# ewrfcas/LeftRefill

Hardware: AMD Instinct MI355X
Metric: 512x1024 stitched images/sec @ 50 DDIM steps, cfg=2.5; per-UNet-step ms (higher is better)
Workload: dtype f16; 1 GPU; configs[1]: 1-ref inpainting, 512x1024 canvas (latent 64x128), B=4 per GPU (UNet batch 8 under CFG), 50 DDIM steps, cfg=2.5, eta=1.0, fp16; global_batch=4, per_gpu_batch=4, ddim_steps=50, parallelism=dp1 (sample-sharded, no data-path collective), ranks=1

## Files before the change

include/leftrefill_hip.h:

```cpp
#ifndef LEFTREFILL_HIP_H
#define LEFTREFILL_HIP_H

#include <stdint.h>

#ifdef __cplusplus
extern "C" {
#endif

#define LR_E_ARG (-1)
#define LR_E_ALIGN (-2)
#define LR_E_UNSUPPORTED (-3)

typedef void* lr_stream_t;
typedef uint16_t lr_half;
#define LR_DTYPE_F16 0
#define LR_DTYPE_BF16 1
#define LR_PIPE_DEFAULT 0
#define LR_PIPE_W8_DEEP 4
#define LR_PIPE_HALO 8

int lr_abi_version(void);

int lr_nchw_f32_to_nhwc_f16(const float* x1, int C1, const float* x2, int C2, lr_half* y, int Cpad, int N, int H,
                            int W, lr_stream_t s);
// ... 45 lines not shown
  int32_t dtype;
  int32_t pipe;
  float* gn_group_out; int32_t gn_hw;
  int32_t wt_bstride, bias_bstride;
  int32_t wt_pm;
  const lr_half* skip1; const lr_half* skip2; int32_t Cs1, Cs2;
  int32_t splitk_mode;
} lr_gemm_args;
int lr_gemm_gn_group_chunks(const lr_gemm_args* args);
int lr_gemm_gn_rows(const lr_gemm_args* args);
int lr_gemm_plan(const lr_gemm_args* args, int32_t* plan);
int lr_gemm_stats_parts(const lr_gemm_args* args);
int64_t lr_gemm_workspace_bytes(const lr_gemm_args* args);
int lr_gemm_conv_f16(const lr_gemm_args* args, lr_stream_t s);
int lr_gemm_splitk_timeouts(void);

int lr_attention_f16(const lr_half* q, int ldq, const lr_half* k, int ldk, const lr_half* v, int ldv, lr_half* o,
                     int ldo, int B, int heads, int Nq, int Nkv, float scale, lr_stream_t s);

int lr_attention_causal_f16(const lr_half* q, int ldq, const lr_half* k, int ldk, const lr_half* v, int ldv, lr_half* o,
                            int ldo, int B, int heads, int N, float scale, lr_stream_t s);
int lr_attention_vt_f16(const lr_half* q, int ldq, const lr_half* k, int ldk, const lr_half* vt, int ld_vt, lr_half* o,
                        int ldo, int B, int heads, int Nq, int Nkv, float scale, lr_stream_t s);
int lr_transpose_v_f16(const lr_half* v, int ldv, lr_half* vt, int ld_vt, int B, int heads, int Nkv, lr_stream_t s);

typedef struct lr_xattn_args {
  const lr_half* x; lr_half* out;
  const lr_half* wq; const float* bq;
  const lr_half* k; int32_t ldk;
  const lr_half* vt;
// ... 215 lines not shown
```

leftrefill_amd/_lib.py:

```python
import ctypes
import os

HERE = os.path.dirname(os.path.abspath(__file__))
LIB_PATH = os.environ.get("LEFTREFILL_LIB_PATH") or os.path.join(HERE, "lib", "libleftrefill_hip.so")
ABI_VERSION = 30

c_void_p, c_int, c_float, c_int64 = ctypes.c_void_p, ctypes.c_int, ctypes.c_float, ctypes.c_int64


class GemmArgs(ctypes.Structure):
    _fields_ = [
        ("p1", c_void_p), ("C1", ctypes.c_int32),
        ("p2", c_void_p), ("C2", ctypes.c_int32),
        ("B", ctypes.c_int32), ("H", ctypes.c_int32), ("W", ctypes.c_int32),
        ("Hs", ctypes.c_int32), ("Ws", ctypes.c_int32),
        ("taps", ctypes.c_int32), ("stride", ctypes.c_int32), ("up", ctypes.c_int32),
        ("asym", ctypes.c_int32),
        ("wt", c_void_p), ("N", ctypes.c_int32),
        ("bias", c_void_p),
        ("rowvec", c_void_p), ("ld_rowvec", ctypes.c_int32),
        ("resid", c_void_p), ("ld_resid", ctypes.c_int32),
        ("out", c_void_p), ("ld_out", ctypes.c_int32),
        ("geglu", ctypes.c_int32),
        ("tile_n", ctypes.c_int32),
        ("tile_m", ctypes.c_int32),
        ("splits", ctypes.c_int32),
        ("workspace", c_void_p), ("workspace_bytes", ctypes.c_int64),
        ("ln_stats", c_void_p), ("ln_parts", ctypes.c_int32), ("ln_eps", ctypes.c_float),
        ("ln_colsum", c_void_p),
        ("stats_out", c_void_p),
        ("gn_stats_out", c_void_p),
        ("dtype", ctypes.c_int32),
        ("pipe", ctypes.c_int32),
        ("gn_group_out", c_void_p), ("gn_hw", ctypes.c_int32),
        ("wt_bstride", ctypes.c_int32), ("bias_bstride", ctypes.c_int32),
        ("wt_pm", ctypes.c_int32),
        ("skip1", c_void_p), ("skip2", c_void_p), ("Cs1", ctypes.c_int32), ("Cs2", ctypes.c_int32),
        ("splitk_mode", ctypes.c_int32),
    ]


class AttnBwdArgs(ctypes.Structure):
    _fields_ = ([(n, c_void_p) for n in ("q", "k", "v", "o", "dout", "qt", "kt", "dot", "lse", "dsum", "dq", "dk", "dv")] +
                [(n, ctypes.c_int32) for n in ("ldq", "ldk", "ldv", "ldo", "lddo", "ld_qt", "ld_kt", "lddq", "lddk", "lddv",
                                               "B", "heads", "Nq", "Nkv")] + [("scale", ctypes.c_float)])


class XattnArgs(ctypes.Structure):
    _fields_ = [("x", c_void_p), ("out", c_void_p), ("wq", c_void_p), ("bq", c_void_p), ("k", c_void_p), ("ldk", ctypes.c_int32),
                ("vt", c_void_p), ("wo", c_void_p), ("bo", c_void_p), ("stats_out", c_void_p),
                ("M", ctypes.c_int32), ("HW", ctypes.c_int32), ("C", ctypes.c_int32), ("heads", ctypes.c_int32),
                ("Lc", ctypes.c_int32), ("ln_eps", ctypes.c_float), ("scale", ctypes.c_float),
                ("pre_a", c_void_p), ("pre_w", c_void_p), ("pre_b", c_void_p)]

# ... 86 lines not shown
    "lr_ddim_cfg_step": [c_void_p, c_void_p, c_int, c_void_p, c_void_p, c_void_p, c_int64, c_float, c_float, c_float,
                         c_float, c_float, c_void_p],
    "lr_timestep_embedding_f32": [c_void_p, c_int, c_int, c_void_p, c_void_p],
    "lr_plms_cfg_step": [c_void_p, c_void_p, c_int, c_void_p, c_int, c_void_p, c_float, c_void_p, c_void_p, c_void_p, c_int64,
                         c_float, c_float, c_float, c_float, c_void_p],
    "lr_dpmpp_cfg_step": [c_void_p, c_void_p, c_int, c_void_p, c_void_p, c_void_p, c_int64, c_float, c_float, c_float, c_float,
                          c_float, c_float, c_float, c_void_p],
    "lr_ddim_inv_cfg_step": [c_void_p, c_void_p, c_int, c_void_p, c_int64, c_float, c_float, c_float, c_void_p],
    "lr_ddim_cfg3_step": [c_void_p, c_void_p, c_int, c_void_p, c_void_p, c_void_p, c_int64, c_float, c_float, c_float, c_float,
                          c_float, c_float, c_float, c_void_p],
    "lr_ddpm_step": [c_void_p, c_void_p, c_int, c_void_p, c_void_p, c_void_p, c_void_p, c_int64, c_int64, c_int, c_void_p, c_void_p,
                     c_int64, c_float, c_float, c_float, c_float, c_float, c_float, c_float, c_void_p],
    "lr_ddim_q_sample": [c_void_p, c_void_p, c_void_p, c_int, c_int64, c_void_p, c_void_p, c_void_p],
    "lr_eval_metrics": [c_void_p, c_int, c_void_p, c_void_p, c_int, c_int, c_int, c_int, c_int, c_int, c_void_p, c_void_p, c_void_p,
                        c_void_p],
}

BF16_TWINS = ["lr_groupnorm_stats", "lr_groupnorm_apply", "lr_groupnorm_apply_n", "lr_layernorm", "lr_layernorm_bwd",
              "lr_groupnorm_bwd", "lr_layernorm_bwd_res", "lr_groupnorm_bwd_res", "lr_nchw_f32_to_nhwc_f16", "lr_nhwc_f16_to_nchw", "lr_timestep_embedding", "lr_linear_small_m",
              "lr_mv_gather", "lr_mv_scatter", "lr_ddim_cfg_step", "lr_timestep_embedding_f32", "lr_plms_cfg_step",
              "lr_dpmpp_cfg_step", "lr_ddim_inv_cfg_step", "lr_ddim_cfg3_step", "lr_ddpm_step", "lr_geglu_fwd", "lr_geglu_bwd", "lr_sumpool2x2",
              "lr_mv_gather_bwd", "lr_mv_scatter_bwd", "lr_attention_f16", "lr_attention_causal_f16", "lr_attention_lse_f16",
              "lr_attention_vt_f16", "lr_transpose_v_f16", "lr_attention_bwd_f16", "lr_xattn_block_f16",
              "lr_xattn_pack_vt_f16", "lr_ffn_block_f16", "lr_stin_block_f16", "lr_rowlin_f16", "lr_gn_conv_out_f16",
              "lr_attention_causal_lse_f16", "lr_attention_causal_bwd_f16", "lr_gelu_fwd_f16", "lr_gelu_bwd_f16"]


def twin(name):
    return (name[:-4] if name.endswith("_f16") else name) + "_bf16"

# ... 67 lines not shown
```

leftrefill_amd/csrc/gemm_conv.hip:

```cpp
#include "gemm_common.h"
#include <atomic>

#ifdef LR_GEMM_TRACE
static unsigned long long* g_trace = nullptr;
extern "C" void lr_gemm_set_trace(void* p) { g_trace = (unsigned long long*)p; }
#endif


template <int BN, int MODE, typename T>
__global__ __launch_bounds__(GEMM_THREADS, BN == 64 ? 4 : BN == 128 ? 3 : 2) void gemm_conv_kernel(const GemmParams P) {
#if defined(__HIP_DEVICE_COMPILE__)
  constexpr int TM = 4;
  constexpr int TN = BN / 32;
  constexpr int A_BYTES = BM * 128;
  constexpr int B_BYTES = BN * 128;
  constexpr int STAGE = A_BYTES + B_BYTES;
  extern __shared__ __attribute__((aligned(16))) char smem[];

  const int t = threadIdx.x;
  const int lane = t & 63;
  const int w = __builtin_amdgcn_readfirstlane(t >> 6);
  const int wm = w >> 1, wn = w & 1;
#ifdef LR_GEMM_STAGGER
  if (P.stagger) {
// ... 622 lines not shown
      if (t < 2 * (8 * RED_GROUPS / gcg)) {
        const int gl = t >> 1, j = t & 1;
        const int g = (blockIdx.x * 8 * RED_GROUPS) / gcg + gl;
        if (g < 32) {
          float a = 0.f;
          for (int c = 0; c < gcg; ++c) a += red[j][gl * gcg + c];
          const int m0 = blockIdx.y * RED_ROWS;
          const int smp = m0 / P.gp_hw, chunk = (m0 - smp * P.gp_hw) / RED_ROWS;
          P.gp_out[(((size_t)smp * P.gp_chunks + chunk) * 32 + g) * 2 + j] = a;
        }
      }
    }
  }
}

template <int BN, int MODE, typename T>
static int launch_gemm_t(const GemmParams& P0, hipStream_t st) {
  GemmParams P = P0;
  P.ntiles_n = (P.N + BN - 1) / BN;
  const int ntm = (P.M + BM - 1) / BM;
  P.ntiles_m = ntm;
  P.m_fastest = 0;
  P.nblocks = P.ntiles_n * ntm;
  const size_t smem = 2 * (size_t)(BM + BN) * 128 + BM * 2 * sizeof(float) + 2 * (((BN + 63) / 64) * 64) * sizeof(float);
  static unsigned long long attr_done = 0;
  if (lr_attr_needed(&attr_done)) {
    hipFuncSetAttribute(reinterpret_cast<const void*>(gemm_conv_kernel<BN, MODE, T>), hipFuncAttributeMaxDynamicSharedMemorySize,
                        (int)smem);
  }
  hipLaunchKernelGGL((gemm_conv_kernel<BN, MODE, T>), dim3(P.nblocks, P.splits), dim3(GEMM_THREADS), smem, st, P);
// ... 147 lines not shown
  if (!base[dev]) {
    void* p = nullptr;
    if (hipGetSymbolAddress(&p, HIP_SYMBOL(lr_sk_counters)) != hipSuccess) return nullptr;
    base[dev] = (unsigned*)p;
  }
  return base[dev] + (size_t)(next.fetch_add(1, std::memory_order_relaxed) & 15) * 2048;
}

extern "C" int lr_gemm_splitk_timeouts(void) {
  unsigned v = 0;
  if (hipMemcpyFromSymbol(&v, HIP_SYMBOL(lr_sk_error), sizeof(v)) != hipSuccess) return -1;
  const unsigned h = lr_halo_sk_timeouts();
  return h == 0xFFFFFFFFu ? -1 : (int)(v + h);
}

extern "C" int lr_gemm_conv_f16(const lr_gemm_args* a, lr_stream_t s) {
  if (!a || !a->p1 || !a->wt || !a->out) return LR_E_ARG;
  GemmParams P;
  P.p1 = (const f16*)a->p1; P.C1 = a->C1;
  P.p2 = (const f16*)a->p2; P.C2 = a->p2 ? a->C2 : 0;
  P.c16 = (P.C1 == 16 && P.C2 == 0 && a->taps == 9 && a->stride == 1 && a->up == 0 && !a->asym) ? 1 : 0;
  if (P.C1 <= 0 || (!P.c16 && P.C1 % 64) || P.C2 % 64) return LR_E_ALIGN;
  if (a->taps != 1 && a->taps != 9) return LR_E_UNSUPPORTED;
  if (a->stride != 1 && a->stride != 2) return LR_E_UNSUPPORTED;
  if (a->up < 0 || a->up > 2) return LR_E_UNSUPPORTED;
  if (a->B <= 0 || a->H <= 0 || a->W <= 0 || a->Hs <= 0 || a->Ws <= 0 || a->N <= 0) return LR_E_ARG;
  P.H = a->H; P.W = a->W; P.Hs = a->Hs; P.Ws = a->Ws;
  P.taps = a->taps; P.stride = a->stride; P.up = a->up;
  P.zins = (a->up == 2) ? 1 : 0;
  if (P.zins) P.up = 1;
  P.pad = a->asym ? 0 : 1;
  P.wt = (const f16*)a->wt; P.N = a->N; P.bias = a->bias;
// ... 79 lines not shown
    if (P.gp_chunks <= 0 || ((uintptr_t)P.gp_out & 7) || a->stats_out) return LR_E_ARG;
    P.gp_cg = P.N / 32;
    P.gp_hw = a->gn_hw > 0 ? a->gn_hw : a->H * a->W;
  }
  P.wt_pm = a->wt_pm ? 1 : 0;
  if (P.wt_pm && (a->wt_bstride || P.K % 64)) return LR_E_ARG;
  P.wt_bstride = a->wt_bstride; P.bias_bstride = a->bias_bstride;
  if (P.wt_bstride) {
    if (a->taps != 1 || splits > 1 || P.rows_per_batch % tm || P.wt_bstride < 0 || P.bias_bstride < 0 || (P.wt_bstride & 7)) return LR_E_ARG;
    if ((int64_t)a->B * P.wt_bstride * 2 >= lim) return LR_E_UNSUPPORTED;
  }
  P.st_out = a->stats_out;
  P.st_parts = ((P.N + tn - 1) / tn) * tile_wnw(tm, tn, P.geglu);
  if (P.st_out && (splits > 1 || ((uintptr_t)P.st_out & 7))) return LR_E_ARG;
  hipStream_t st = (hipStream_t)s;
  int rc;
  const int mode = P.geglu ? 1 : P.gelu ? 2 : 0;
  if (a->pipe != 0 && a->pipe != choose_stages(tm, tn, a->pipe)) return LR_E_UNSUPPORTED;
  const bool deep = tm == 128 && choose_stages(tm, tn, a->pipe) == 4;
#ifdef LR_DEV_VARIANTS
  if (P.splits > 1 && a->splitk_mode == 1 && mode != 1 && (tn == 160 || tn == 320) && (tm == 256 || deep || a->pipe == LR_PIPE_HALO)) {
    const int64_t tiles = (int64_t)((P.M + tm - 1) / tm) * ((P.N + tn - 1) / tn);
    if (tiles * P.splits <= 256 && tiles <= 2048 && (int64_t)P.splits * P.M * P.N * 4 < lim && P.N % 8 == 0)
      P.sk_cnt = sk_counter_slot();
  }
#endif
  if (a->pipe == LR_PIPE_HALO) {
    if (mode != 0 || a->asym) return LR_E_UNSUPPORTED;
    rc = lr_launch_conv_halo(P, tn, st);
    if (rc || P.splits == 1 || P.sk_cnt) return rc;
    return launch_reduce(P, st);
  }
  if (mode == 0) {
    if (deep && tn == 128) rc = launch_pipe<128, 8, 128, 4, 4, 0>(P, st);
    else if (deep && tn == 160) rc = launch_pipe<128, 8, 160, 4, 4, 0>(P, st);

    else if (tm == 128 && tn == 128) rc = launch_gemm<128, 0>(P, st);
    else if (tm == 128 && tn == 64) rc = launch_gemm<64, 0>(P, st);
    else if (tm == 128 && tn == 160) rc = launch_gemm<160, 0>(P, st);
    else if (tm == 256 && tn == 128) rc = launch_gemm256<128, 4, 3, 0>(P, st);
    else if (tm == 256 && tn == 160) rc = launch_gemm256<160, 4, 3, 0>(P, st);
    else if (tm == 256 && tn == 256) rc = launch_gemm256<256, 2, 2, 0>(P, st);
    else if (tm == 256 && tn == 320) rc = launch_gemm256<320, 2, 2, 0>(P, st);
    else return LR_E_UNSUPPORTED;
  } else if (mode == 1) {
    if (deep && tn == 128) rc = launch_pipe<128, 8, 128, 4, 4, 1>(P, st);
    else if (deep) return LR_E_UNSUPPORTED;
    else if (tm == 128 && tn == 128) rc = launch_gemm<128, 1>(P, st);
    else if (tm == 128 && tn == 64) rc = launch_gemm<64, 1>(P, st);
    else if (tm == 256 && tn == 128) rc = launch_gemm256<128, 4, 3, 1>(P, st);
    else if (tm == 256 && tn == 256) rc = launch_gemm256<256, 2, 2, 1>(P, st);
    else if (tm == 256 && tn == 320) rc = launch_gemm256<320, 4, 2, 1>(P, st);
    else return LR_E_UNSUPPORTED;
  } else {
    if (deep) return LR_E_UNSUPPORTED;
    if (tm == 128 && tn == 128) rc = launch_gemm<128, 2>(P, st);
    else if (tm == 128 && tn == 64) rc = launch_gemm<64, 2>(P, st);
    else if (tm == 256 && tn == 128) rc = launch_gemm256<128, 4, 3, 2>(P, st);
    else return LR_E_UNSUPPORTED;
  }
  if (rc || P.splits == 1 || P.sk_cnt) return rc;
  return launch_reduce(P, st);
}
```

leftrefill_amd/csrc/stin_block.hip:

```cpp
#include "chain_common.h"

#define SI_C 320
#define SI_ROWS 256
#define SI_THREADS 512
#define SI_SLOT 40960
#define SI_OUT_AUX 0

struct StinParams {
  const void* x; const void* wp; const float* bp; const void* wqkv; const float* bqkv;
  void* x1; void* qkv;
  int M, NQ, ld_qkv;
  float eps;
  const float* gn_part; const float* gn_gamma; const float* gn_beta; int gn_chunks, gn_hw; float gn_eps;
#ifdef SI_TRACE
  unsigned long long* trace;
#endif
};

#ifdef SI_TRACE
#define SI_STAMP(k) do { if (P.trace && lane == 0) P.trace[((size_t)blockIdx.x * 8 + w) * 64 + (k)] = __builtin_readcyclecounter(); } while (0)
static unsigned long long* g_si_trace = nullptr;
extern "C" void lr_stin_set_trace(void* p) { g_si_trace = (unsigned long long*)p; }
#else
#define SI_STAMP(k) do { } while (0)
// ... 231 lines not shown
  if ((int64_t)a->NQ * SI_C * 2 >= ((int64_t)1 << 31)) return LR_E_UNSUPPORTED;
  StinParams P;
  P.x = a->x; P.wp = a->wp; P.bp = a->bp; P.wqkv = a->wqkv; P.bqkv = a->bqkv; P.x1 = a->x1; P.qkv = a->qkv;
  P.M = a->M; P.NQ = a->NQ; P.ld_qkv = a->ld_qkv; P.eps = a->ln_eps;
  const bool gn = a->gn_part != nullptr;
  if (gn) {
    if (!a->gn_gamma || !a->gn_beta || a->gn_chunks <= 0 || a->gn_hw <= 0) return LR_E_ARG;
    if (a->gn_hw % SI_ROWS || a->M % a->gn_hw) return LR_E_UNSUPPORTED;
    if (((uintptr_t)a->gn_part & 7) || (((uintptr_t)a->gn_gamma | (uintptr_t)a->gn_beta) & 3)) return LR_E_ALIGN;
  }
  P.gn_part = a->gn_part; P.gn_gamma = a->gn_gamma; P.gn_beta = a->gn_beta; P.gn_chunks = a->gn_chunks; P.gn_hw = a->gn_hw; P.gn_eps = a->gn_eps;
#ifdef SI_TRACE
  P.trace = g_si_trace;
#endif
  const size_t smem = 3 * SI_SLOT + (size_t)(SI_C + a->NQ + 2 * SI_C + 64) * sizeof(float);
  static unsigned long long attr_done[2] = {0, 0};
  if (gn) {
    if (lr_attr_needed(&attr_done[1]))
      hipFuncSetAttribute(reinterpret_cast<const void*>(stin_block_kernel<T, true>), hipFuncAttributeMaxDynamicSharedMemorySize, (int)smem);
    hipLaunchKernelGGL((stin_block_kernel<T, true>), dim3(a->M / SI_ROWS), dim3(SI_THREADS), smem, (hipStream_t)s, P);
  } else {
    if (lr_attr_needed(&attr_done[0]))
      hipFuncSetAttribute(reinterpret_cast<const void*>(stin_block_kernel<T, false>), hipFuncAttributeMaxDynamicSharedMemorySize, (int)smem);
    hipLaunchKernelGGL((stin_block_kernel<T, false>), dim3(a->M / SI_ROWS), dim3(SI_THREADS), smem, (hipStream_t)s, P);
  }
  return lr_launch_status();
}

extern "C" int lr_stin_block_f16(const lr_stin_args* a, lr_stream_t s) { return stin_block_t<f16>(a, s); }
extern "C" int lr_stin_block_bf16(const lr_stin_args* a, lr_stream_t s) { return stin_block_t<bf16>(a, s); }
```

leftrefill_amd/engine.py:

```python
import math
from dataclasses import dataclass
from typing import Optional

import torch

from . import packing
from . import train_ops as ops
from .ops import plan_batch_scale

_COMPUTE = [torch.float16]


def compute_dtype():
    return _COMPUTE[0]


class compute:

    def __init__(self, dtype):
        if dtype not in (torch.float16, torch.bfloat16):
            raise ValueError(f"compute dtype must be float16 or bfloat16, got {dtype}")
        self.dtype = dtype

    def __enter__(self):
# ... 1 lines not shown
        _COMPUTE[0] = self.dtype

    def __exit__(self, *exc):
        _COMPUTE[0] = self.prev


@dataclass
class Act:
    tok: torch.Tensor
    N: int
    H: int
    W: int
    tok2: Optional[torch.Tensor] = None
    gs: Optional[tuple] = None
    gs2: Optional[tuple] = None

    @property
    def HW(self):
        return self.H * self.W

    def materialize(self):
        if self.tok2 is None:
            return self.tok
        return torch.cat([self.tok, self.tok2], dim=1).contiguous()


def f32(p):
    return p.detach().float().contiguous()


# ... 163 lines not shown


def ln_linear(x, st, pn: PackedNorm, pl: PackedLinear, wide=None):
    if wide and pl.wf is not None and fold_ok(x) and ops.rowlin_ok(x.shape[0], x.shape[1], pl.wf.shape[0], wide):
        return ops.rowlin(x, pl.wf, pl.bf, eps=pl.eps)
    if st is not None and pl.wf is not None and fold_ok(x):
        return ops.gemm_conv(x, pl.wf, B=1, H=1, W=x.shape[0], taps=1, bias=pl.bf, ln=(st, pl.eps, pl.cs))
    return linear(ops.layer_norm(x, pn.g, pn.b, pn.eps), pl)


GN_FUSE = __import__("os").environ.get("LEFTREFILL_GN_FUSE", "1") != "0"
SKIP_FUSED = __import__("os").environ.get("LEFTREFILL_SKIP_FUSED", "1") != "0"
FF_PROJ = __import__("os").environ.get("LEFTREFILL_FF_PROJ", "1") != "0"


def gn_fuse_ok(x):
    return GN_FUSE and not (torch.is_grad_enabled() and x.requires_grad)


TRAIN_GN_STATS = __import__("os").environ.get("LEFTREFILL_TRAIN_GN_STATS", "1") != "0"
TRAIN_FORK = __import__("os").environ.get("LEFTREFILL_TRAIN_FORK", "1") != "0"


TRAIN_SKIP_FUSED = __import__("os").environ.get("LEFTREFILL_TRAIN_SKIP_FUSED", "1") != "0"


def gn_stats_ok(x):
    return GN_FUSE and (TRAIN_GN_STATS or not torch.is_grad_enabled())


def training(x):
    return torch.is_grad_enabled() and x.requires_grad


def forking(x):
    return TRAIN_FORK and training(x)


def conv(act: Act, pc: PackedConv, rowvec=None, resid=None, up=0, asym=False, gn_stats=False, skip=None, skip_parts=None):
    if pc.taps == 9:
        if up:
            H, W = act.H * 2, act.W * 2
        elif pc.stride == 2:
            H, W = act.H // 2, act.W // 2
        else:
            H, W = act.H, act.W
    else:
        H, W = act.H, act.W
    want = gn_stats and gn_stats_ok(act.tok) and pc.cout == pc.w.shape[0]
    extra = {} if skip_parts is None else {"skip_parts": skip_parts}
    y = ops.gemm_conv(act.tok, pc.w, B=act.N, H=H, W=W, Hs=act.H, Ws=act.W, taps=pc.taps, stride=pc.stride, up=up,
                      asym=asym, x2=act.tok2, bias=pc.b, rowvec=rowvec, resid=resid, want_gn_stats=want, skip=skip, **extra)
    y, gs = y if want else (y, None)
    return Act(y, act.N, H, W, gs=gs)


def _gn_train_stats(act: Act):
    HW = act.HW
    if not (act.gs is not None and HW % act.gs[1] == 0 and gn_stats_ok(act.tok)
            and (act.tok2 is None or (act.gs2 is not None and HW % act.gs2[1] == 0))):
        return None
    if act.tok2 is None and act.gs[2] is not None:
        return ("groups", act.gs[2], act.gs[3])
    return ("channels", act.gs, act.gs2)


def gn(act: Act, pn: PackedNorm, silu):
    HW = act.HW
    if training(act.tok) or (act.tok2 is not None and training(act.tok2)):
        return Act(ops.group_norm(act.tok, act.N, HW, pn.g, pn.b, pn.eps, silu, act.tok2, stats=_gn_train_stats(act)), act.N, act.H, act.W)
    fused = (act.gs is not None and HW % act.gs[1] == 0 and gn_fuse_ok(act.tok)
             and (act.tok2 is None or (act.gs2 is not None and HW % act.gs2[1] == 0)))
    if fused and act.tok2 is None and act.gs[2] is not None:
        y = ops.group_norm_groups(act.tok, act.N, HW, pn.g, pn.b, pn.eps, silu, act.gs[2], act.gs[3])
    elif fused:
        y = ops.group_norm_fused(act.tok, act.N, HW, pn.g, pn.b, pn.eps, silu, act.gs, act.tok2, act.gs2)
    else:
        y = ops.group_norm(act.tok, act.N, HW, pn.g, pn.b, pn.eps, silu, act.tok2)
    return Act(y, act.N, act.H, act.W)


def gn_fork(act: Act, pn: PackedNorm, silu):
    y, t1, t2 = ops.group_norm_fork(act.tok, act.N, act.HW, pn.g, pn.b, pn.eps, silu, act.tok2, stats=_gn_train_stats(act))
    return Act(y, act.N, act.H, act.W), Act(t1, act.N, act.H, act.W, tok2=t2)


def resblock(act: Act, pr: PackedRes, emb_out):
    if forking(act.tok) or (act.tok2 is not None and forking(act.tok2)):
        h, act = gn_fork(act, pr.n1, True)
    else:
        h = gn(act, pr.n1, True)
    h = conv(h, pr.c1, rowvec=emb_out, gn_stats=True)
    h = gn(h, pr.n2, True)
    if pr.c2s is not None and SKIP_FUSED and gn_fuse_ok(act.tok) and gn_fuse_ok(h.tok) and (act.tok2 is None or gn_fuse_ok(act.tok2)):
        return conv(h, pr.c2s, gn_stats=True, skip=(act.tok, act.tok2))
    if (pr.c2s is not None and SKIP_FUSED and TRAIN_SKIP_FUSED and (training(h.tok) or training(act.tok) or (act.tok2 is not None and training(act.tok2)))
            and h.tok2 is None):
        return conv(h, pr.c2s, gn_stats=True, skip=(act.tok, act.tok2), skip_parts=(pr.c2.w, pr.skip.w))
    if pr.skip is not None:
        resid = conv(act, pr.skip).tok
    else:
        resid = act.materialize()
    return conv(h, pr.c2, resid=resid, gn_stats=True)


def attention_plain(x, ctx, pa: PackedAttn, B, L, Lc=None):
    if pa.is_self:
# ... 336 lines not shown
```

leftrefill_amd/ops.py:

```python
import ctypes
import os

import torch

from . import _lib
from ._lib import FfnArgs, GemmArgs, RowlinArgs, StinArgs, XattnArgs

GN_CHUNKS = 256
GN_GROUPS = os.environ.get("LEFTREFILL_GN_GROUPS", "1") != "0"

AUTOTUNE = os.environ.get("LEFTREFILL_AUTOTUNE", "0") == "1"
TILE_CANDIDATES = ((128, 64, 0), (128, 128, 0), (128, 160, 0), (128, 128, 4), (128, 160, 4), (256, 128, 0), (256, 160, 0),
                   (256, 256, 0), (256, 320, 0), (256, 160, 8), (256, 320, 8))
TILE_TABLE_PATH = os.environ.get("LEFTREFILL_TILE_TABLE_PATH",
                                 os.path.join(os.path.dirname(os.path.abspath(__file__)), "tile_table.json"))
_tile_cache = None
PLAN_LOG = os.environ.get("LEFTREFILL_PLAN_LOG", "0") == "1"
SPLITK_MODE = int(os.environ.get("LEFTREFILL_SPLITK_MODE", "0"))
_untabulated = set()
TABLE_HITS, TABLE_MISSES = set(), set()
PLAN_TRIAL = None
LAUNCH_HOOK = None


# ... 179 lines not shown
    _chk16(a, "a")
    _chk16(w, "w")
    M, K = a.shape
    N = w.shape[0]
    out = torch.empty(M, N, device=a.device, dtype=a.dtype)
    st = _stream()
    for m0 in range(0, M, 16):
        mc = min(16, M - m0)
        _lib.check(_fn(lib, "lr_linear_small_m", a.dtype)(a[m0:].data_ptr(), K, _p(w), _p(bias), out[m0:].data_ptr(), N, mc, N, K,
                                         int(act_in), int(act_out), st), "linear_small_m")
    return out


def gemm_conv(x1, wt, *, B, H, W, Hs=None, Ws=None, taps=1, stride=1, up=0, asym=False, x2=None, bias=None, rowvec=None,
              resid=None, geglu=False, gelu=False, out=None, tile_n=0, tile_m=0, splits=0, pipe=0, ln=None,
              want_stats=False, want_gn_stats=False, gn_hw=0, per_sample=False, wt_pm=False, skip=None):
    lib = _lib.load()
    _chk16(x1, "x1")
    _chk16(wt, "wt")
    Hs = H if Hs is None else Hs
    Ws = W if Ws is None else Ws
    C1 = x1.shape[-1]
    C2 = 0
    if x2 is not None:
        _chk16(x2, "x2")
        C2 = x2.shape[-1]
    if per_sample:
        assert wt.dim() == 3 and wt.shape[0] == B and taps == 1 and x2 is None and wt.is_contiguous() and not wt_pm
    if wt_pm:
        assert wt.dim() == 3 and wt.shape[2] == 64 and wt.is_contiguous()
        Nw, Kw = wt.shape[1], wt.shape[0] * 64
# ... 78 lines not shown
                a.pipe = 0
        if skip is not None and best is None:
            plan = (ctypes.c_int32 * 4)()
            lib.lr_gemm_plan(a, plan)
            a.tile_m, a.tile_n, a.splits, a.pipe = plan[0], plan[1], plan[2], plan[3]
    stats = None
    if want_stats:
        if a.splits == 0:
            a.splits = 1
        parts = lib.lr_gemm_stats_parts(a)
        stats = torch.empty(M, parts, 2, device=x1.device, dtype=torch.float32)
        a.stats_out = _p(stats)
    if ln is not None and a.splits == 0:
        a.splits = 1
    gstats = None
    if want_gn_stats:
        plan = (ctypes.c_int32 * 4)()
        lib.lr_gemm_plan(a, plan)
        a.splits = plan[2]
        rows = lib.lr_gemm_gn_rows(a)
        hw = gn_hw or H * W
        if hw % rows == 0:
            chunks = lib.lr_gemm_gn_group_chunks(a) if GN_GROUPS else 0
            gp = torch.empty(M // hw, chunks, 32, 2, device=x1.device, dtype=torch.float32) if chunks > 0 else None
            gstats = (torch.empty((M + rows - 1) // rows, n_out, 2, device=x1.device, dtype=torch.float32), rows, gp, chunks)
            a.gn_stats_out = _p(gstats[0])
            a.gn_group_out = _p(gp)
    ws = _workspace(lib, a, x1.device)
    if LAUNCH_HOOK is not None and tile_m == 0 and tile_n == 0 and splits == 0:
        plan = (ctypes.c_int32 * 4)()
        lib.lr_gemm_plan(a, plan)
        LAUNCH_HOOK(key, 0, tuple(plan))
        rc = lib.lr_gemm_conv_f16(a, st)
        LAUNCH_HOOK(key, 1, rc)
        if rc != 0 and PLAN_TRIAL is not None and PLAN_TRIAL.get(key) is not None:
            PLAN_TRIAL[key] = None
            return gemm_conv(x1, wt, B=B, H=H, W=W, Hs=Hs, Ws=Ws, taps=taps, stride=stride, up=up, asym=asym, x2=x2, bias=bias, rowvec=rowvec,
                             resid=resid, geglu=geglu, gelu=gelu, out=out, ln=ln, want_stats=want_stats, want_gn_stats=want_gn_stats, gn_hw=gn_hw,
                             per_sample=per_sample, wt_pm=wt_pm, skip=skip)
        _lib.check(rc, "gemm_conv")
    else:
        _lib.check(lib.lr_gemm_conv_f16(a, st), "gemm_conv")
    if want_gn_stats:
        return out, gstats
    return (out, stats) if want_stats else out


HEURISTIC_REFINE = os.environ.get("LEFTREFILL_HEURISTIC_REFINE", "1") != "0"


def _lib_plan(lib, a):
    plan = (ctypes.c_int32 * 4)()
    lib.lr_gemm_plan(a, plan)
    return tuple(plan)


def _refine_plan(lib, a, act_epilogue):
    base = _lib_plan(lib, a)
    tm, tn = base[0], base[1]
    M = a.B * a.H * a.W
# ... 472 lines not shown
```

Baseline: 4.781 images/s.

## Fuse split-K reduction with following GroupNorm+SiLU in ResBlock conv1

Adds a split-K reduce kernel that sums the partials, applies bias, rowvec and residual, keeps the per-sample tile in shared memory, computes GroupNorm statistics and writes the normalized SiLU output directly. ResBlock conv1 uses it when eligible (hw<=512, split-K planned) and skips writing the raw conv output, removing the separate GN apply pass and one activation round trip. The cost is one block per sample per 40 channels, which may limit parallelism, plus double-precision stat reduction. It also raises the stin_block dynamic shared-memory attribute to a fixed maximum.

```diff
diff --git a/include/leftrefill_hip.h b/include/leftrefill_hip.h
--- a/include/leftrefill_hip.h
+++ b/include/leftrefill_hip.h
@@ -83,6 +83,27 @@
 int64_t lr_gemm_workspace_bytes(const lr_gemm_args* args);
 int lr_gemm_conv_f16(const lr_gemm_args* args, lr_stream_t s);
 int lr_gemm_splitk_timeouts(void);
+
+typedef struct lr_reduce_gn_args {
+  const float* partials; int32_t splits, M, N;
+  int32_t hw;
+  const float* bias;
+  const lr_half* rowvec; int32_t ld_rowvec;
+  const lr_half* resid; int32_t ld_resid;
+  lr_half* raw; int32_t ld_raw;
+  const float* gamma; const float* beta; float eps; int32_t silu;
+  lr_half* y;
+  float* gn_group_out;
+  int32_t dtype;
+} lr_reduce_gn_args;
+int lr_splitk_reduce_gn(const lr_reduce_gn_args* args, lr_stream_t s);
+int lr_splitk_reduce(const lr_reduce_gn_args* args, lr_stream_t s);
+typedef struct lr_gn_consumer {
+  const float* gamma; const float* beta; float eps; int32_t silu;
+  lr_half* y;
+} lr_gn_consumer;
+int lr_gemm_conv_gn_f16(const lr_gemm_args* args, const lr_gn_consumer* gn, lr_stream_t s);
+int lr_gemm_reduce_gn_ok(const lr_gemm_args* args);
 
 int lr_attention_f16(const lr_half* q, int ldq, const lr_half* k, int ldk, const lr_half* v, int ldv, lr_half* o,
                      int ldo, int B, int heads, int Nq, int Nkv, float scale, lr_stream_t s);
diff --git a/leftrefill_amd/_lib.py b/leftrefill_amd/_lib.py
--- a/leftrefill_amd/_lib.py
+++ b/leftrefill_amd/_lib.py
@@ -38,6 +38,17 @@
         ("skip1", c_void_p), ("skip2", c_void_p), ("Cs1", ctypes.c_int32), ("Cs2", ctypes.c_int32),
         ("splitk_mode", ctypes.c_int32),
     ]
+
+
+class ReduceGnArgs(ctypes.Structure):
+    _fields_ = [("partials", c_void_p), ("splits", ctypes.c_int32), ("M", ctypes.c_int32), ("N", ctypes.c_int32), ("hw", ctypes.c_int32),
+                ("bias", c_void_p), ("rowvec", c_void_p), ("ld_rowvec", ctypes.c_int32), ("resid", c_void_p), ("ld_resid", ctypes.c_int32),
+                ("raw", c_void_p), ("ld_raw", ctypes.c_int32), ("gamma", c_void_p), ("beta", c_void_p), ("eps", ctypes.c_float),
+                ("silu", ctypes.c_int32), ("y", c_void_p), ("gn_group_out", c_void_p), ("dtype", ctypes.c_int32)]
+
+
+class GnConsumer(ctypes.Structure):
+    _fields_ = [("gamma", c_void_p), ("beta", c_void_p), ("eps", ctypes.c_float), ("silu", ctypes.c_int32), ("y", c_void_p)]
 
 
 class AttnBwdArgs(ctypes.Structure):
@@ -154,6 +165,10 @@
     "lr_ddim_q_sample": [c_void_p, c_void_p, c_void_p, c_int, c_int64, c_void_p, c_void_p, c_void_p],
     "lr_eval_metrics": [c_void_p, c_int, c_void_p, c_void_p, c_int, c_int, c_int, c_int, c_int, c_int, c_void_p, c_void_p, c_void_p,
                         c_void_p],
+    "lr_splitk_reduce_gn": [ctypes.POINTER(ReduceGnArgs), c_void_p],
+    "lr_splitk_reduce": [ctypes.POINTER(ReduceGnArgs), c_void_p],
+    "lr_gemm_conv_gn_f16": [ctypes.POINTER(GemmArgs), ctypes.POINTER(GnConsumer), c_void_p],
+    "lr_gemm_reduce_gn_ok": [ctypes.POINTER(GemmArgs)],
 }
 
 BF16_TWINS = ["lr_groupnorm_stats", "lr_groupnorm_apply", "lr_groupnorm_apply_n", "lr_layernorm", "lr_layernorm_bwd",
diff --git a/leftrefill_amd/csrc/gemm_conv.hip b/leftrefill_amd/csrc/gemm_conv.hip
--- a/leftrefill_amd/csrc/gemm_conv.hip
+++ b/leftrefill_amd/csrc/gemm_conv.hip
@@ -660,6 +660,162 @@
   }
 }
 
+#define RG_OCT 5
+#define RG_CH (8 * RG_OCT)
+#define RG_ROWS 128
+#define RG_THREADS (RG_OCT * RG_ROWS)
+#define RG_MAX_HW 512
+#define RG_MAX_CHUNKS (RG_MAX_HW / RED_ROWS)
+struct ReduceGnParams {
+  const float* ws; int splits, M, N, hw;
+  const float* bias; const void* rowvec; int ld_rowvec; const void* resid; int ld_resid;
+  void* raw; int ld_raw;
+  const float* gamma; const float* beta; float eps; int silu; void* y;
+};
+
+template <typename T>
+__global__ __launch_bounds__(RG_THREADS) void splitk_reduce_gn_kernel(const ReduceGnParams P) {
+  __shared__ uint4 rows[RG_MAX_HW * RG_OCT];
+  __shared__ float chs[RG_MAX_CHUNKS][RG_CH][2];
+  __shared__ float gps[RG_MAX_CHUNKS][4][2];
+  __shared__ float s_mean[4], s_rstd[4];
+  const int t = threadIdx.x, o = t % RG_OCT, r = t / RG_OCT;
+  const int ncb = P.N / RG_CH, total = gridDim.x;
+  const int vb = total % 8 == 0 ? (blockIdx.x % 8) * (total / 8) + blockIdx.x / 8 : blockIdx.x;
+  const int smp = vb / ncb, n = (vb - smp * ncb) * RG_CH + o * 8;
+  const int Cg = P.N / 32, ngl = RG_CH / Cg, nchunks = P.hw / RED_ROWS;
+  const size_t slice = (size_t)P.M * P.N;
+  const T* rowvec = (const T*)P.rowvec;
+  const T* resid = (const T*)P.resid;
+  float add[8];
+  float rv[8];
+#pragma unroll
+  for (int i = 0; i < 8; ++i) { add[i] = P.bias ? P.bias[n + i] : 0.f; rv[i] = 0.f; }
+  if (rowvec) lr_unpack8<T>(*reinterpret_cast<const uint4*>(rowvec + (size_t)smp * P.ld_rowvec + n), rv);
+  for (int row = r; row < P.hw; row += RG_ROWS) {
+    const size_t m = (size_t)smp * P.hw + row;
+    const float* src = P.ws + m * P.N + n;
+    float v[8];
+#pragma unroll
+    for (int i = 0; i < 8; ++i) v[i] = 0.f;
+    int sidx = 0;
+    for (; sidx + 4 <= P.splits; sidx += 4) {
+      f32x4 a[4], b[4];
+#pragma unroll
+      for (int k = 0; k < 4; ++k) {
+        a[k] = *reinterpret_cast<const f32x4*>(src + (sidx + k) * slice);
+        b[k] = *reinterpret_cast<const f32x4*>(src + (sidx + k) * slice + 4);
+      }
+#pragma unroll
+      for (int k = 0; k < 4; ++k) {
+        v[0] += a[k][0]; v[1] += a[k][1]; v[2] += a[k][2]; v[3] += a[k][3];
+        v[4] += b[k][0]; v[5] += b[k][1]; v[6] += b[k][2]; v[7] += b[k][3];
+      }
+    }
+    for (; sidx < P.splits; ++sidx) {
+      const f32x4 a = *reinterpret_cast<const f32x4*>(src + sidx * slice), b = *reinterpret_cast<const f32x4*>(src + sidx * slice + 4);
+      v[0] += a[0]; v[1] += a[1]; v[2] += a[2]; v[3] += a[3]; v[4] += b[0]; v[5] += b[1]; v[6] += b[2]; v[7] += b[3];
+    }
+    if (P.bias) {
+#pragma unroll
+      for (int i = 0; i < 8; ++i) v[i] += add[i];
+    }
+    if (rowvec) {
+#pragma unroll
+      for (int i = 0; i < 8; ++i) v[i] += rv[i];
+    }
+    if (resid) {
+      float e[8];
+      lr_unpack8<T>(*reinterpret_cast<const uint4*>(resid + m * P.ld_resid + n), e);
+#pragma unroll
+      for (int i = 0; i < 8; ++i) v[i] += e[i];
+    }
+    const uint4 pk = lr_pack8<T>(v);
+    rows[row * RG_OCT + o] = pk;
+    if (P.raw) *reinterpret_cast<uint4*>((T*)P.raw + m * P.ld_raw + n) = pk;
+  }
+  __syncthreads();
+  {
+#pragma clang fp contract(off)
+    const T* hv = reinterpret_cast<const T*>(rows);
+    for (int e = t; e < nchunks * RG_CH; e += RG_THREADS) {
+      const int c = e / RG_CH, ch = e - c * RG_CH;
+      float s = 0.f, q = 0.f;
+#pragma unroll 8
+      for (int k = 0; k < RED_ROWS; ++k) {
+        const float x = (float)hv[(size_t)(c * RED_ROWS + k) * RG_CH + ch];
+        const float xx = x * x;
+        s += x; q += xx;
+      }
+      chs[c][ch][0] = s; chs[c][ch][1] = q;
+    }
+  }
+  __syncthreads();
+  for (int e = t; e < nchunks * ngl * 2; e += RG_THREADS) {
+    const int j = e & 1, gl = (e >> 1) % ngl, c = (e >> 1) / ngl;
+    float a = 0.f;
+    for (int cc = 0; cc < Cg; ++cc) a += chs[c][gl * Cg + cc][j];
+    gps[c][gl][j] = a;
+  }
+  __syncthreads();
+  if (t < 4 * ngl) {
+    const int g = t >> 2, sub = t & 3;
+    double s = 0.0, q = 0.0;
+#pragma unroll 4
+    for (int c = sub; c < nchunks; c += 4) { s += (double)gps[c][g][0]; q += (double)gps[c][g][1]; }
+#pragma unroll
+    for (int sh = 2; sh > 0; sh >>= 1) { s += __shfl_xor(s, sh, 64); q += __shfl_xor(q, sh, 64); }
+    if (sub == 0) {
+      const double cnt = (double)P.hw * (double)Cg;
+      const double mean = s / cnt;
+      double var = q / cnt - mean * mean;
+      if (var < 0.0) var = 0.0;
+      s_mean[g] = (float)mean;
+      s_rstd[g] = (float)(1.0 / sqrt(var + (double)P.eps));
+    }
+  }
+  __syncthreads();
+  float a[8], b[8];
+#pragma unroll
+  for (int i = 0; i < 8; ++i) {
+    const int g = (o * 8 + i) / Cg;
+    const float ga = P.gamma[n + i], be = P.beta[n + i];
+    a[i] = s_rstd[g] * ga;
+    b[i] = be - s_mean[g] * a[i];
+  }
+  const int silu = P.silu;
+  T* dst = (T*)P.y + ((size_t)smp * P.hw) * P.N + n;
+  for (int row = r; row < P.hw; row += RG_ROWS) {
+    float f[8];
+    lr_unpack8<T>(rows[row * RG_OCT + o], f);
+#pragma unroll
+    for (int i = 0; i < 8; ++i) {
+      const float z = fmaf(f[i], a[i], b[i]);
+      f[i] = silu ? z * __builtin_amdgcn_rcpf(1.0f + __expf(-z)) : z;
+    }
+    *reinterpret_cast<uint4*>(dst + (size_t)row * P.N) = lr_pack8<T>(f);
+  }
+}
+
+static int reduce_gn_check(const ReduceGnParams& R) {
+  if (!R.ws || !R.gamma || !R.beta || !R.y || R.splits < 2 || R.M <= 0 || R.N <= 0 || R.hw <= 0) return LR_E_ARG;
+  if (R.N % 32 || R.N % RG_CH || RG_CH % (R.N / 32)) return LR_E_UNSUPPORTED;
+  if (R.hw % RED_ROWS || R.hw > RG_MAX_HW || R.M % R.hw || R.M / R.hw > 65535) return LR_E_UNSUPPORTED;
+  if ((R.rowvec && R.ld_rowvec % 8) || (R.resid && R.ld_resid % 8) || (R.raw && R.ld_raw % 8)) return LR_E_ALIGN;
+  if (((uintptr_t)R.ws | (uintptr_t)R.bias | (uintptr_t)R.rowvec | (uintptr_t)R.resid | (uintptr_t)R.raw | (uintptr_t)R.y) & 15) return LR_E_ALIGN;
+  if (((uintptr_t)R.gamma | (uintptr_t)R.beta) & 3) return LR_E_ALIGN;
+  return 0;
+}
+
+static int launch_reduce_gn(const ReduceGnParams& R, int bf16_, hipStream_t st) {
+  const int rc = reduce_gn_check(R);
+  if (rc) return rc;
+  const dim3 grid((R.N / RG_CH) * (R.M / R.hw));
+  if (bf16_) hipLaunchKernelGGL(splitk_reduce_gn_kernel<bf16>, grid, dim3(RG_THREADS), 0, st, R);
+  else hipLaunchKernelGGL(splitk_reduce_gn_kernel<f16>, grid, dim3(RG_THREADS), 0, st, R);
+  return lr_launch_status();
+}
+
 template <int BN, int MODE, typename T>
 static int launch_gemm_t(const GemmParams& P0, hipStream_t st) {
   GemmParams P = P0;
@@ -837,8 +993,8 @@
   return h == 0xFFFFFFFFu ? -1 : (int)(v + h);
 }
 
-extern "C" int lr_gemm_conv_f16(const lr_gemm_args* a, lr_stream_t s) {
-  if (!a || !a->p1 || !a->wt || !a->out) return LR_E_ARG;
+static int gemm_conv_impl(const lr_gemm_args* a, const lr_gn_consumer* g, lr_stream_t s) {
+  if (!a || !a->p1 || !a->wt || (!a->out && !g)) return LR_E_ARG;
   GemmParams P;
   P.p1 = (const f16*)a->p1; P.C1 = a->C1;
   P.p2 = (const f16*)a->p2; P.C2 = a->p2 ? a->C2 : 0;
@@ -948,6 +1104,16 @@
   P.st_parts = ((P.N + tn - 1) / tn) * tile_wnw(tm, tn, P.geglu);
   if (P.st_out && (splits > 1 || ((uintptr_t)P.st_out & 7))) return LR_E_ARG;
   hipStream_t st = (hipStream_t)s;
+  ReduceGnParams R = {};
+  if (g) {
+    if (splits <= 1 || P.geglu || P.gelu || a->splitk_mode != 0 || P.gs_out || P.gp_out || P.st_out || P.ln_part) return LR_E_ARG;
+    R.ws = P.ws; R.splits = splits; R.M = P.M; R.N = P.N; R.hw = P.rows_per_batch;
+    R.bias = P.bias; R.rowvec = P.rowvec; R.ld_rowvec = P.ld_rowvec; R.resid = P.resid; R.ld_resid = P.ld_resid;
+    R.raw = P.out; R.ld_raw = P.ld_out;
+    R.gamma = g->gamma; R.beta = g->beta; R.eps = g->eps; R.silu = g->silu; R.y = g->y;
+    const int rcg = reduce_gn_check(R);
+    if (rcg) return rcg;
+  }
   int rc;
   const int mode = P.geglu ? 1 : P.gelu ? 2 : 0;
   if (a->pipe != 0 && a->pipe != choose_stages(tm, tn, a->pipe)) return LR_E_UNSUPPORTED;
@@ -963,7 +1129,7 @@
     if (mode != 0 || a->asym) return LR_E_UNSUPPORTED;
     rc = lr_launch_conv_halo(P, tn, st);
     if (rc || P.splits == 1 || P.sk_cnt) return rc;
-    return launch_reduce(P, st);
+    return g ? launch_reduce_gn(R, P.bf16, st) : launch_reduce(P, st);
   }
   if (mode == 0) {
     if (deep && tn == 128) rc = launch_pipe<128, 8, 128, 4, 4, 0>(P, st);
@@ -994,5 +1160,56 @@
     else return LR_E_UNSUPPORTED;
   }
   if (rc || P.splits == 1 || P.sk_cnt) return rc;
-  return launch_reduce(P, st);
-}
+  return g ? launch_reduce_gn(R, P.bf16, st) : launch_reduce(P, st);
+}
+
+extern "C" int lr_gemm_conv_f16(const lr_gemm_args* a, lr_stream_t s) { return gemm_conv_impl(a, nullptr, s); }
+
+extern "C" int lr_gemm_conv_gn_f16(const lr_gemm_args* a, const lr_gn_consumer* g, lr_stream_t s) {
+  if (!g) return LR_E_ARG;
+  return gemm_conv_impl(a, g, s);
+}
+
+extern "C" int lr_gemm_reduce_gn_ok(const lr_gemm_args* a) {
+  if (!a || a->geglu || a->splitk_mode != 0 || a->gn_stats_out || a->gn_group_out || a->stats_out || a->ln_stats) return 0;
+  int32_t plan[4];
+  if (lr_gemm_plan(a, plan) || plan[2] <= 1) return 0;
+  const int hw = a->H * a->W, N = a->N;
+  if (N % 32 || N % RG_CH || RG_CH % (N / 32)) return 0;
+  if (hw <= 0 || hw % RED_ROWS || hw > RG_MAX_HW || a->B > 65535) return 0;
+  return 1;
+}
+
+static int reduce_args(const lr_reduce_gn_args* a, ReduceGnParams* R) {
+  if (!a || (a->dtype != LR_DTYPE_F16 && a->dtype != LR_DTYPE_BF16)) return LR_E_ARG;
+  *R = ReduceGnParams{};
+  R->ws = a->partials; R->splits = a->splits; R->M = a->M; R->N = a->N; R->hw = a->hw;
+  R->bias = a->bias; R->rowvec = a->rowvec; R->ld_rowvec = a->ld_rowvec; R->resid = a->resid; R->ld_resid = a->ld_resid;
+  R->raw = a->raw; R->ld_raw = a->ld_raw;
+  R->gamma = a->gamma; R->beta = a->beta; R->eps = a->eps; R->silu = a->silu; R->y = a->y;
+  return 0;
+}
+
+extern "C" int lr_splitk_reduce_gn(const lr_reduce_gn_args* a, lr_stream_t s) {
+  ReduceGnParams R;
+  const int rc = reduce_args(a, &R);
+  if (rc) return rc;
+  return launch_reduce_gn(R, a->dtype == LR_DTYPE_BF16, (hipStream_t)s);
+}
+
+extern "C" int lr_splitk_reduce(const lr_reduce_gn_args* a, lr_stream_t s) {
+  if (!a || !a->partials || !a->raw || a->splits < 1 || a->M <= 0 || a->N <= 0 || a->hw <= 0 || a->M % a->hw) return LR_E_ARG;
+  if (a->dtype != LR_DTYPE_F16 && a->dtype != LR_DTYPE_BF16) return LR_E_ARG;
+  if (a->N % 8 || a->ld_raw % 8 || (a->resid && a->ld_resid % 8) || (a->rowvec && a->ld_rowvec % 8)) return LR_E_ALIGN;
+  if (((uintptr_t)a->partials | (uintptr_t)a->bias | (uintptr_t)a->rowvec | (uintptr_t)a->resid | (uintptr_t)a->raw) & 15) return LR_E_ALIGN;
+  GemmParams P = {};
+  P.ws = (float*)a->partials; P.splits = a->splits; P.M = a->M; P.N = a->N; P.rows_per_batch = a->hw;
+  P.bias = a->bias; P.rowvec = (const f16*)a->rowvec; P.ld_rowvec = a->ld_rowvec; P.resid = (const f16*)a->resid; P.ld_resid = a->ld_resid;
+  P.out = (f16*)a->raw; P.ld_out = a->ld_raw; P.bf16 = a->dtype == LR_DTYPE_BF16;
+  P.gp_out = a->gn_group_out; P.gp_cg = 1; P.gp_hw = 1;
+  if (P.gp_out) {
+    if (a->N % 32 || (8 * RED_GROUPS) % (a->N / 32) || a->hw % RED_ROWS || ((uintptr_t)P.gp_out & 7)) return LR_E_ARG;
+    P.gp_cg = a->N / 32; P.gp_hw = a->hw; P.gp_chunks = a->hw / RED_ROWS;
+  }
+  return launch_reduce(P, (hipStream_t)s);
+}
diff --git a/leftrefill_amd/csrc/stin_block.hip b/leftrefill_amd/csrc/stin_block.hip
--- a/leftrefill_amd/csrc/stin_block.hip
+++ b/leftrefill_amd/csrc/stin_block.hip
@@ -269,14 +269,15 @@
   P.trace = g_si_trace;
 #endif
   const size_t smem = 3 * SI_SLOT + (size_t)(SI_C + a->NQ + 2 * SI_C + 64) * sizeof(float);
+  const int smem_max = (int)(3 * SI_SLOT + (size_t)(SI_C + 4096 + 2 * SI_C + 64) * sizeof(float));
   static unsigned long long attr_done[2] = {0, 0};
   if (gn) {
     if (lr_attr_needed(&attr_done[1]))
-      hipFuncSetAttribute(reinterpret_cast<const void*>(stin_block_kernel<T, true>), hipFuncAttributeMaxDynamicSharedMemorySize, (int)smem);
+      hipFuncSetAttribute(reinterpret_cast<const void*>(stin_block_kernel<T, true>), hipFuncAttributeMaxDynamicSharedMemorySize, smem_max);
     hipLaunchKernelGGL((stin_block_kernel<T, true>), dim3(a->M / SI_ROWS), dim3(SI_THREADS), smem, (hipStream_t)s, P);
   } else {
     if (lr_attr_needed(&attr_done[0]))
-      hipFuncSetAttribute(reinterpret_cast<const void*>(stin_block_kernel<T, false>), hipFuncAttributeMaxDynamicSharedMemorySize, (int)smem);
+      hipFuncSetAttribute(reinterpret_cast<const void*>(stin_block_kernel<T, false>), hipFuncAttributeMaxDynamicSharedMemorySize, smem_max);
     hipLaunchKernelGGL((stin_block_kernel<T, false>), dim3(a->M / SI_ROWS), dim3(SI_THREADS), smem, (hipStream_t)s, P);
   }
   return lr_launch_status();
diff --git a/leftrefill_amd/engine.py b/leftrefill_amd/engine.py
--- a/leftrefill_amd/engine.py
+++ b/leftrefill_amd/engine.py
@@ -39,6 +39,7 @@
     tok2: Optional[torch.Tensor] = None
     gs: Optional[tuple] = None
     gs2: Optional[tuple] = None
+    pre: Optional[tuple] = None
 
     @property
     def HW(self):
@@ -232,6 +233,9 @@
 FF_PROJ = __import__("os").environ.get("LEFTREFILL_FF_PROJ", "1") != "0"
 
 
+REDUCE_GN = ops.REDUCE_GN
+
+
 def gn_fuse_ok(x):
     return GN_FUSE and not (torch.is_grad_enabled() and x.requires_grad)
 
@@ -255,7 +259,8 @@
     return TRAIN_FORK and training(x)
 
 
-def conv(act: Act, pc: PackedConv, rowvec=None, resid=None, up=0, asym=False, gn_stats=False, skip=None, skip_parts=None):
+def conv(act: Act, pc: PackedConv, rowvec=None, resid=None, up=0, asym=False, gn_stats=False, skip=None, skip_parts=None, gn_next=None,
+         keep_raw=True):
     if pc.taps == 9:
         if up:
             H, W = act.H * 2, act.W * 2
@@ -267,6 +272,12 @@
         H, W = act.H, act.W
     want = gn_stats and gn_stats_ok(act.tok) and pc.cout == pc.w.shape[0]
     extra = {} if skip_parts is None else {"skip_parts": skip_parts}
+    if gn_next is not None and want and gn_fuse_ok(act.tok) and skip_parts is None:
+        pn, silu = gn_next
+        y, gs, yn = ops.gemm_conv(act.tok, pc.w, B=act.N, H=H, W=W, Hs=act.H, Ws=act.W, taps=pc.taps, stride=pc.stride, up=up,
+                                  asym=asym, x2=act.tok2, bias=pc.b, rowvec=rowvec, resid=resid, want_gn_stats=True, skip=skip,
+                                  gn_next=(pn.g, pn.b, pn.eps, silu, keep_raw))
+        return Act(y, act.N, H, W, gs=gs, pre=None if yn is None else (pn, bool(silu), yn))
     y = ops.gemm_conv(act.tok, pc.w, B=act.N, H=H, W=W, Hs=act.H, Ws=act.W, taps=pc.taps, stride=pc.stride, up=up,
                       asym=asym, x2=act.tok2, bias=pc.b, rowvec=rowvec, resid=resid, want_gn_stats=want, skip=skip, **extra)
     y, gs = y if want else (y, None)
@@ -285,6 +296,8 @@
 
 def gn(act: Act, pn: PackedNorm, silu):
     HW = act.HW
+    if act.pre is not None and act.pre[0] is pn and act.pre[1] == bool(silu) and act.tok2 is None:
+        return Act(act.pre[2], act.N, act.H, act.W)
     if training(act.tok) or (act.tok2 is not None and training(act.tok2)):
         return Act(ops.group_norm(act.tok, act.N, HW, pn.g, pn.b, pn.eps, silu, act.tok2, stats=_gn_train_stats(act)), act.N, act.H, act.W)
     fused = (act.gs is not None and HW % act.gs[1] == 0 and gn_fuse_ok(act.tok)
@@ -308,7 +321,7 @@
         h, act = gn_fork(act, pr.n1, True)
     else:
         h = gn(act, pr.n1, True)
-    h = conv(h, pr.c1, rowvec=emb_out, gn_stats=True)
+    h = conv(h, pr.c1, rowvec=emb_out, gn_stats=True, gn_next=(pr.n2, True) if REDUCE_GN else None, keep_raw=False)
     h = gn(h, pr.n2, True)
     if pr.c2s is not None and SKIP_FUSED and gn_fuse_ok(act.tok) and gn_fuse_ok(h.tok) and (act.tok2 is None or gn_fuse_ok(act.tok2)):
         return conv(h, pr.c2s, gn_stats=True, skip=(act.tok, act.tok2))
diff --git a/leftrefill_amd/ops.py b/leftrefill_amd/ops.py
--- a/leftrefill_amd/ops.py
+++ b/leftrefill_amd/ops.py
@@ -217,7 +217,7 @@
 
 def gemm_conv(x1, wt, *, B, H, W, Hs=None, Ws=None, taps=1, stride=1, up=0, asym=False, x2=None, bias=None, rowvec=None,
               resid=None, geglu=False, gelu=False, out=None, tile_n=0, tile_m=0, splits=0, pipe=0, ln=None,
-              want_stats=False, want_gn_stats=False, gn_hw=0, per_sample=False, wt_pm=False, skip=None):
+              want_stats=False, want_gn_stats=False, gn_hw=0, per_sample=False, wt_pm=False, skip=None, gn_next=None):
     lib = _lib.load()
     _chk16(x1, "x1")
     _chk16(wt, "wt")
@@ -326,36 +326,94 @@
     if ln is not None and a.splits == 0:
         a.splits = 1
     gstats = None
+    gn_y = gnc = None
+    assert gn_next is None or want_gn_stats
     if want_gn_stats:
         plan = (ctypes.c_int32 * 4)()
         lib.lr_gemm_plan(a, plan)
         a.splits = plan[2]
         rows = lib.lr_gemm_gn_rows(a)
         hw = gn_hw or H * W
-        if hw % rows == 0:
+        if (gn_next is not None and REDUCE_GN and not gn_hw and not geglu and not gelu and out.is_contiguous()
+                and lib.lr_gemm_reduce_gn_ok(a) == 1):
+            gamma, beta, geps, silu, keep_raw = gn_next
+            assert gamma.dtype == torch.float32 and beta.dtype == torch.float32 and gamma.numel() == n_out and beta.numel() == n_out
+            gn_y = torch.empty(M, n_out, device=x1.device, dtype=x1.dtype)
+            gnc = _lib.GnConsumer(_p(gamma), _p(beta), float(geps), int(bool(silu)), _p(gn_y))
+            if not keep_raw:
+                out, a.out = None, 0
+        elif hw % rows == 0:
             chunks = lib.lr_gemm_gn_group_chunks(a) if GN_GROUPS else 0
             gp = torch.empty(M // hw, chunks, 32, 2, device=x1.device, dtype=torch.float32) if chunks > 0 else None
             gstats = (torch.empty((M + rows - 1) // rows, n_out, 2, device=x1.device, dtype=torch.float32), rows, gp, chunks)
             a.gn_stats_out = _p(gstats[0])
             a.gn_group_out = _p(gp)
     ws = _workspace(lib, a, x1.device)
+
+    def launch():
+        return lib.lr_gemm_conv_f16(a, st) if gnc is None else lib.lr_gemm_conv_gn_f16(a, ctypes.byref(gnc), st)
+
     if LAUNCH_HOOK is not None and tile_m == 0 and tile_n == 0 and splits == 0:
         plan = (ctypes.c_int32 * 4)()
         lib.lr_gemm_plan(a, plan)
         LAUNCH_HOOK(key, 0, tuple(plan))
-        rc = lib.lr_gemm_conv_f16(a, st)
+        rc = launch()
         LAUNCH_HOOK(key, 1, rc)
         if rc != 0 and PLAN_TRIAL is not None and PLAN_TRIAL.get(key) is not None:
             PLAN_TRIAL[key] = None
             return gemm_conv(x1, wt, B=B, H=H, W=W, Hs=Hs, Ws=Ws, taps=taps, stride=stride, up=up, asym=asym, x2=x2, bias=bias, rowvec=rowvec,
                              resid=resid, geglu=geglu, gelu=gelu, out=out, ln=ln, want_stats=want_stats, want_gn_stats=want_gn_stats, gn_hw=gn_hw,
-                             per_sample=per_sample, wt_pm=wt_pm, skip=skip)
+                             per_sample=per_sample, wt_pm=wt_pm, skip=skip, gn_next=gn_next)
         _lib.check(rc, "gemm_conv")
     else:
-        _lib.check(lib.lr_gemm_conv_f16(a, st), "gemm_conv")
+        _lib.check(launch(), "gemm_conv")
+    if gn_next is not None:
+        return out, gstats, gn_y
     if want_gn_stats:
         return out, gstats
     return (out, stats) if want_stats else out
+
+
+REDUCE_GN = os.environ.get("LEFTREFILL_REDUCE_GN", "1") != "0"
+
+
+def _reduce_gn_args(partials, hw, bias, rowvec, resid, raw, dtype):
+    splits, M, N = partials.shape
+    assert partials.dtype == torch.float32 and partials.is_contiguous() and M % hw == 0
+    a = _lib.ReduceGnArgs()
+    a.partials, a.splits, a.M, a.N, a.hw = _p(partials), splits, M, N, hw
+    a.bias = _p(bias)
+    a.rowvec, a.ld_rowvec = _p(rowvec), (rowvec.stride(0) if rowvec is not None else 0)
+    a.resid, a.ld_resid = _p(resid), (resid.stride(0) if resid is not None else 0)
+    a.raw, a.ld_raw = _p(raw), (raw.stride(0) if raw is not None else 0)
+    a.dtype = int(dtype == torch.bfloat16)
+    for t_ in (rowvec, resid):
+        assert t_ is None or t_.dtype == dtype
+    assert bias is None or (bias.dtype == torch.float32 and bias.numel() == N)
+    return a
+
+
+def splitk_reduce(partials, hw, dtype, bias=None, rowvec=None, resid=None):
+    lib = _lib.load()
+    _, M, N = partials.shape
+    raw = torch.empty(M, N, device=partials.device, dtype=dtype)
+    gp = torch.empty(M // hw, hw // 32, 32, 2, device=partials.device, dtype=torch.float32)
+    a = _reduce_gn_args(partials, hw, bias, rowvec, resid, raw, dtype)
+    a.gn_group_out = _p(gp)
+    _lib.check(lib.lr_splitk_reduce(a, _stream()), "splitk_reduce")
+    return raw, gp
+
+
+def splitk_reduce_gn(partials, hw, dtype, gamma, beta, eps, silu, bias=None, rowvec=None, resid=None, keep_raw=False):
+    lib = _lib.load()
+    _, M, N = partials.shape
+    raw = torch.empty(M, N, device=partials.device, dtype=dtype) if keep_raw else None
+    y = torch.empty(M, N, device=partials.device, dtype=dtype)
+    a = _reduce_gn_args(partials, hw, bias, rowvec, resid, raw, dtype)
+    assert gamma.dtype == torch.float32 and beta.dtype == torch.float32 and gamma.numel() == N and beta.numel() == N
+    a.gamma, a.beta, a.eps, a.silu, a.y = _p(gamma), _p(beta), float(eps), int(bool(silu)), _p(y)
+    _lib.check(lib.lr_splitk_reduce_gn(a, _stream()), "splitk_reduce_gn")
+    return raw, y
 
 
 HEURISTIC_REFINE = os.environ.get("LEFTREFILL_HEURISTIC_REFINE", "1") != "0"
```

Result: no change. 4.796 images/s (median of 6 runs) (+0.3%).
